# AdaptiveCity/deepdish

Hardware: AMD Instinct MI355X
Metric: end-to-end frames/sec (detect+encode+track) at 640x480 (higher is better)
Workload: dtype i8 (reference: uint8); encoder f16; 1 GPU; SSD-MobileNet-v1 uint8-quantised (300x300) + MARS-64x32x3 + deep_sort on synthetic 640x480 BGR frames, ~20 synthetic detections/frame (BASELINE.json configs[1]); streams_per_gpu=3072, worker_threads_per_gpu=2, parallelism=independent streams, 3072 per GPU in 2 worker groups, weights=seeded synthetic (seed 1234)

## Files before the change

### deepdish_amd/_lib.py

```python
import ctypes
import os
from ctypes import c_int, c_int64, c_double, c_float, c_void_p, c_char_p, POINTER

HERE = os.path.dirname(os.path.abspath(__file__))
LIB_PATH = os.environ.get('DD_LIB') or os.path.join(HERE, 'libdeepdish_hip.so')

P = c_void_p


class DeepDishHipError(RuntimeError):
    pass


SIGNATURES = {
    'dd_last_error': [],
    'dd_version': [],
    'dd_ctx_create': [c_int, POINTER(P)],
    'dd_ctx_destroy': [P],
    'dd_ctx_stream': [P, POINTER(P)],
    'dd_ctx_sync': [P],
    'dd_kf_initiate': [P, P, P, P, P, c_int, P],
    'dd_kf_predict': [P, P, P, P, c_int, P],
    'dd_kf_project': [P, P, P, P, c_int, P, P, P],
    'dd_kf_update': [P, P, P, P, P, c_int, P],
# ... 44 lines not shown
    'dd_ingest_create_jpeg_scaled': [P, c_int, c_int, c_int, c_int, c_int, c_int, c_int, c_int, c_int64, P],
    'dd_ingest_jpeg_put': [P, c_int, c_int, P, c_int64],
    'dd_ingest_create_jpeg_ex': [P, c_int, c_int, c_int, c_int, c_int, c_int, c_int, c_int, c_int, c_int64, P],
    'dd_ingest_status': [P, c_int, P],
    'dd_ingest_destroy': [P],
    'dd_ingest_host_slot': [P, c_int, P, P],
    'dd_ingest_submit': [P, c_int],
    'dd_ingest_wait_uploaded': [P, c_int],
    'dd_ingest_acquire': [P, c_int, P, P],
    'dd_ingest_release': [P, c_int, P],
    'dd_mog2_create': [P, c_int, c_int, c_int, c_int, c_double, c_int, POINTER(P)],
    'dd_mog2_destroy': [P],
    'dd_mog2_state': [P, c_int, P, P, P, P],
    'dd_mog2_apply': [P, P, c_double, P, P, P],
    'dd_mog2_apply_streams': [P, P, P, c_double, P, P, P],
    'dd_mask_box_count': [P, P, c_int, c_int, c_int, P, P, c_int, P, P],
    'dd_net_create': [P, P, c_int, P, c_int64, c_int, POINTER(P)],
    'dd_net_create_shared': [P, P, c_int, P, c_int64, c_int, POINTER(P)],
    'dd_net_activation_bytes': [P, POINTER(c_int64)],
    'dd_net_destroy': [P],
    'dd_net_forward': [P, P, c_int, P],
    'dd_net_output': [P, c_int, POINTER(P), POINTER(c_int), POINTER(c_int), POINTER(c_int), POINTER(c_int),
                      POINTER(c_int)],
    'dd_net_use_graph': [P, c_int],
    'dd_net_input_size': [P, POINTER(c_int), POINTER(c_int)],
    'dd_net_max_batch': [P, POINTER(c_int)],
    'dd_net_last_batch': [P, POINTER(c_int)],
    'dd_net_read': [P, c_int, c_int, P, c_int, P],
    'dd_net_profile': [P, c_int],
    'dd_net_profile_read': [P, P, c_int, POINTER(c_int)],
    'dd_net_op_launches': [P, P, c_int, POINTER(c_int)],
    'dd_net_op_variants': [P, P, c_int, POINTER(c_int)],
    'dd_netq_dwpw_fits': [c_int, c_int, c_int, c_int, c_int, c_int, POINTER(c_int)],
    'dd_ssd_postprocess': [P, P, P, c_int, c_int, c_int, c_float, c_float, P, P, P, P, P],
    'dd_ssd_decode': [P, P, P, c_int, c_int, c_float, P, P, P, P, c_int, P],
    'dd_ssd_postprocess_decoded': [P, P, P, P, P, c_int, c_int, c_float, c_float, P, P, P, P, c_int, P],
    'dd_ssd_regular_nms_decoded': [P, P, P, c_int, c_int, c_int, c_int, c_int, c_int, c_float, c_float, P, P, P, P, c_int, P],
    'dd_ssd_postprocess_regular': [P, P, P, c_int, c_int, c_int, c_int, c_float, c_float, P, P, P, P, c_int, P],
    'dd_ssd_postprocess_regular_u8': [P, P, P, c_int, P, P, P, c_int, c_int, c_int, c_int, c_float, c_float, P, P, P, P, c_int, P],
    'dd_net_ssd_heads_u8': [P, POINTER(P), POINTER(P), POINTER(c_int), POINTER(P), P, POINTER(c_int), POINTER(c_int)],
    'dd_net_ssd_decode': [P, P, c_int, c_float, c_int],
    'dd_net_ssd_decoded': [P, POINTER(P), POINTER(P), POINTER(P), POINTER(P)],
    'dd_net_ssd_decoded_read': [P, c_int, P, P, P, P],
    'dd_net_yolo_decode': [P, c_int],
    'dd_net_yolo_decoded': [P, P, P, P, P],
    'dd_net_yolo_decoded_read': [P, c_int, P, P, P],
    'dd_ssd_detections': [P, P, P, P, c_int, c_int, c_double, c_double, c_double, c_double, P, P, P, P, P],
    'dd_yolov5_decode': [P, P, c_int, c_int, c_float, c_float, c_float, P, P, P, c_int, P, P],
    'dd_yolov5_decode_letterbox': [P, P, c_int, c_int, c_float, c_int, c_int, c_int, c_int, P, P, P, c_int, P, P],
    'dd_pipeline_create': [P, c_int, c_int, c_int, P, P, c_int, c_int, P, c_char_p, c_char_p, c_double, c_double,
                           c_double, c_int, c_int, P, c_int, c_int, POINTER(P)],
    'dd_pipeline_destroy': [P],
    'dd_pipeline_detector_adaptor': [P, c_int],
    'dd_pipeline_ssd_options': [P, c_int, c_float, c_float],
    'dd_pipeline_ssd_regular_nms': [P, c_int],
    'dd_pipeline_detector_skip_frames': [P, c_int],
    'dd_pipeline_detector_letterbox': [P, c_int],
    'dd_pipeline_metric': [P, c_int],
    'dd_pipeline_association': [P, c_int],
    'dd_pipeline_step': [P, P, P, P, P, P],
    'dd_pipeline_step2': [P, P, P, P, P, P, P],
    'dd_pipeline_step3': [P, P, P, P, P, P, P, P, P],
    'dd_pipeline_frames_seen': [P, P],
    'dd_pipeline_present_stats': [P, P],
    'dd_pipeline_detector_skip_streams': [P, P, P],
    'dd_pipeline_skip_stats': [P, P, P],
# ... 97 lines not shown
```

### deepdish_amd/csrc/netsq.hip

```cpp
#include <algorithm>
#include <atomic>
#include <cstdlib>
#include <type_traits>
#include "common.h"
#include "ssd_dev.h"
#include "net_priv.h"
#include "netsq_dev.h"

namespace {


struct QConvP {
    const uint8_t *in; int H, W, c16_in;
    int kh, kw, stride, off_y, off_x;
    int ho, wo, m;
    const i4v *w;
    const int *cbias;
    int kc_per_tap, n_mfrag, mq;
    uint8_t *out; int epi;
    int Ho, Wo, c16_out;
    long long img_bytes_out; int row_bytes, base_off, cout_store;
    int zwc;
    unsigned hw_magic, wo_magic;
    QReq R;
// ... 433 lines not shown
        const u4v v = *reinterpret_cast<const u4v *>(c + sub * 16);
#pragma unroll
        for (int i = 0; i < 16; ++i) {
            const int k = sub * 16 + i;
            const int q = lut[(v[i >> 2] >> (8 * (i & 3))) & 0xffu];
            if (k >= 1 && k < P.n_classes && q > best) { best = q; bi = k - 1; }
        }
    }
#pragma unroll
    for (int o = 4; o > 0; o >>= 1) {
        const int ob = __shfl_xor(best, o, 64), oi = __shfl_xor(bi, o, 64);
        if (ob > best || (ob == best && oi < bi)) { best = ob; bi = oi; }
    }
    if (live && sub == 0) {
#pragma clang fp contract(off)
        const uint8_t *b = P.box + (z * P.n_anchors + a) * 4;
        float r[4], an[4], bx[4];
#pragma unroll
        for (int q = 0; q < 4; ++q) { r[q] = P.box_scale * ((float)b[q] - P.box_zp); an[q] = P.anchors[a * 4 + q]; }
        (void)ssddev::decode_anchor(r, an, 0.f, bx);
        const float sc = P.sc_scale * ((float)best - P.sc_zp);
        const size_t o = z * P.n_anchors + a;
#pragma unroll
        for (int q = 0; q < 4; ++q) P.boxes[o * 4 + q] = bx[q];
        P.score[o] = sc;
        P.cls_out[o] = bi;
        P.keys[o] = sc >= P.thr ? sc : -1.f;
    }
}

struct QDwpwP {
    const uint8_t *in; int H, W;
    int off_y, off_x, ho, wo, hw, tiles_per_frame;
    uint8_t *out; int c16_out;
    const uint2 *dw_a;
    const long long *dw_cq;
    const i4v *w;
    const i4v *w2;
    const int *cbias;
    const long long *cq;
    int zwc, NR;
    int dup;
    unsigned wo_magic, nr_magic, tpf_magic;
    unsigned long long *dbg;
    QReq Rd, Rp;
};

constexpr int QT = 64;

template <int CIN, int COUT, int WP, int STRIDE, int LPT, bool ROWSUM, int MW = 4, int SAT = 0, bool HL = false, int QTT = QT>
__global__ __launch_bounds__((COUT / (16 * MW)) * WP * 64, (COUT / (16 * MW)) * WP <= 2 ? 3 : QTT > 64 ? 4 : 2) void q_dwpw_k(const QDwpwP P, const int n_tiles, const int tiles_per_block) {
    constexpr int WM = COUT / (16 * MW), NW = WM * WP, NT = NW * 64;
    static_assert(MW == 4 || MW == 2, "fragments per wave");
    static_assert(!(HL && ROWSUM), "the split filter needs no row sums");
    constexpr int KC = (CIN + 63) / 64, CINP = KC * 64, C16 = CIN / 16;
    constexpr int FPT = QTT / 16, UNITS = C16 * (FPT / 4);
    static_assert(QTT % 64 == 0 && UNITS % NW == 0, "depthwise units over waves");
    constexpr int CPW = UNITS / NW;
    static_assert(FPT == 4 || CPW == 1, "several units per wave: one fragment quad only");
    constexpr bool KEEP = CPW <= 2, FOLDP = !ROWSUM && KC <= 4 && QTT == 64;
    extern __shared__ __attribute__((aligned(16))) uint8_t smem[];
    const int tid = threadIdx.x, lane = tid & 63, wave = __builtin_amdgcn_readfirstlane(tid >> 6);
    const int fr = lane & 15, fq = lane >> 4;
    const int wm = wave / WP, wp = wave % WP;
    const int RB = (P.W + 2) * CIN, PP = (P.W + 2) * 16;
    uint8_t *opnd = smem;
    int *rowsum = reinterpret_cast<int *>(opnd + QTT * CINP);
    i4v *pinfo = reinterpret_cast<i4v *>(rowsum + 2 * QTT);
    int *cbl = reinterpret_cast<int *>(pinfo + 2 * QTT);
    uint2 *dwa_l = reinterpret_cast<uint2 *>(cbl + COUT);
    long long *dwq_l = reinterpret_cast<long long *>(dwa_l + (KEEP ? 0 : C16 * 64));
    uint8_t *ring = reinterpret_cast<uint8_t *>(dwq_l + (KEEP ? 0 : CIN));

    i4v Wr[MW][KC];
#pragma unroll
    for (int m = 0; m < MW; ++m)
#pragma unroll
        for (int kc = 0; kc < KC; ++kc) Wr[m][kc] = P.w[((size_t)(wm * MW + m) * KC + kc) * 64 + lane];
    const int mg = (wm * MW) / 4, m0 = (wm * MW) % 4;
    unsigned wlm = 0;
    int kcl = -1;
    i4v Wl1[HL ? MW : 1];
    if constexpr (HL) {
// ... 31 lines not shown
    int tap_dx[3];
#pragma unroll
    for (int ks = 0; ks < 3; ++ks) tap_dx[ks] = (min(4 * ks + fq, 8) % 3) * 16;
    const bool row_up0 = fq == 3, row_up1 = fq >= 2;
    auto build_a = [&](int cg, i4v (&Ah)[3], unsigned &lo_w, long long (&Cq)[4], unsigned &lom) {
        const uint2 ab = P.dw_a[cg * 64 + lane];
        lo_w = ab.y;
        lom = (unsigned)__builtin_amdgcn_readfirstlane((int)(ab.y >> 24));
#pragma unroll
        for (int ks = 0; ks < 3; ++ks) {
            const unsigned rh = __builtin_amdgcn_perm(ab.x, ab.x, 0x01010101u * (unsigned)ks);
#pragma unroll
            for (int d = 0; d < 4; ++d) Ah[ks][d] = (int)(rh & dmask[d]);
        }
#pragma unroll
        for (int r = 0; r < 4; ++r) Cq[r] = P.dw_cq[cg * 16 + 4 * fq + r];
    };
    i4v KAh[KEEP ? CPW : 1][3];
    long long KCq[KEEP ? CPW : 1][4];
    unsigned Klom[KEEP ? CPW : 1] = {}, Klow[KEEP ? CPW : 1] = {};
    if constexpr (KEEP) {
#pragma unroll
        for (int ci = 0; ci < CPW; ++ci) build_a((wave * CPW + ci) % C16, KAh[ci], Klow[ci], KCq[ci], Klom[ci]);
    }

    const int t_begin = blockIdx.x * tiles_per_block, t_end = min(n_tiles, t_begin + tiles_per_block);
    if (t_begin >= t_end) return;
    const int Md = P.Rd.M, shd = P.Rd.e - 1, Mp = P.Rp.M, shp = P.Rp.e - 1;
    const long long Cp = P.Rp.C;
    const int lod = P.Rd.lo, hid = P.Rd.hi, lop = P.Rp.lo, hip_ = P.Rp.hi;
    const int out_row = P.c16_out * ((P.wo + 2) * 16);
    const unsigned ring_bytes = (unsigned)P.NR * (unsigned)RB;

    auto tile_rows = [&](int t, int &n, int &q0, int &q1, int &ga, int &gb) {
        n = (int)__umulhi((unsigned)t, P.tpf_magic);
        q0 = (t - n * P.tiles_per_frame) * QTT;
        q1 = min(q0 + QTT, P.hw) - 1;
        const int y0 = (int)__umulhi((unsigned)q0, P.wo_magic), y1 = (int)__umulhi((unsigned)q1, P.wo_magic);
        ga = n * (P.H + 2) + y0 * STRIDE + P.off_y;
        gb = n * (P.H + 2) + y1 * STRIDE + P.off_y + 2;
    };
    auto geometry = [&](int n, int q0, int q1, int ga, int buf) {
        const int q = q0 + tid;
        const int qc = min(q, q1);
        const int y = (int)__umulhi((unsigned)qc, P.wo_magic), x = qc - __mul24(y, P.wo);
        const int y0 = (int)__umulhi((unsigned)q0, P.wo_magic);
        const int sa = ga - (int)__umulhi((unsigned)ga, P.nr_magic) * P.NR;
        int s0 = sa + (y - y0) * STRIDE;
        s0 = s0 >= P.NR ? s0 - P.NR : s0;
        const int s1 = s0 + 1 == P.NR ? 0 : s0 + 1, s2 = s1 + 1 == P.NR ? 0 : s1 + 1;
        const int col = (x * STRIDE + P.off_x) * 16;
        const unsigned po = q <= q1 ? (unsigned)__mul24(n * (P.ho + 2) + y + 1, out_row) + (unsigned)(x + 1) * 16u : 0xffffffffu;
        pinfo[buf * QTT + tid] = i4v{__mul24(s0, RB) + col, __mul24(s1, RB) + col, __mul24(s2, RB) + col, (int)po};
    };
    auto load_rows_sync = [&](int lo, int hi) {
        if (hi < lo) return;
        const unsigned nb = (unsigned)(hi - lo + 1) * RB;
        const uint8_t *src = P.in + (size_t)lo * RB;
        for (unsigned idx = tid * 16u; idx < nb; idx += NT * 16u) {
            const unsigned row = idx / (unsigned)RB, off = idx - row * RB;
            *reinterpret_cast<u4v *>(ring + (size_t)((lo + row) % P.NR) * RB + off) = *reinterpret_cast<const u4v *>(src + idx);
        }
    };
    auto dw_planes = [&](int gbuf, int rsb) __attribute__((always_inline)) {
        int rs[4] = {0, 0, 0, 0};
        constexpr int FB = QTT > 64 ? 2 : 4;
        constexpr bool TAP_ONCE = FB == 4;
        int tapoff[3][4];
        const int fb = 4 * ((wave * CPW) / C16);
        auto taps = [&](int f0, int nfr) __attribute__((always_inline)) {
#pragma unroll
            for (int f = 0; f < 4; ++f) {
                if (f < f0 || f >= f0 + nfr) continue;
                const i4v pi = pinfo[gbuf * QTT + 16 * (fb + f) + fr];
                tapoff[0][f] = (row_up0 ? pi[1] : pi[0]) + tap_dx[0];
                tapoff[1][f] = (row_up1 ? pi[2] : pi[1]) + tap_dx[1];
                tapoff[2][f] = pi[2] + tap_dx[2];
            }
        };
        if constexpr (TAP_ONCE) taps(0, 4);
        auto plane = [&](int unit, int ci) __attribute__((always_inline)) {
            const int cg = unit % C16;
            const int pofs = cg * PP;
            uint2 ab = make_uint2(0u, 0u);
            if constexpr (!KEEP) ab = dwa_l[cg * 64 + lane];
// ... 133 lines not shown
                if (fq == 0) atomicAdd(&rowsum[rsb * QTT + 16 * (fb + f) + fr], v);
            }
        }
    };
    auto glds16 = [&](const uint8_t *g, const uint8_t *l) {
        unsigned keep;
        const unsigned dst = (unsigned)(uintptr_t)(const __attribute__((address_space(3))) uint8_t *)l;
        asm volatile("s_mov_b32 %0, m0\n\ts_mov_b32 m0, %2\n\ts_nop 0\n\tglobal_load_lds_dwordx4 %1, off\n\ts_mov_b32 m0, %0"
                     : "=&s"(keep) : "v"(g), "s"(dst) : "memory");
    };
    auto pf_issue = [&](int lo, int hi) {
        if (hi < lo) return;
        const unsigned nb = (unsigned)(hi - lo + 1) * (unsigned)RB;
        const uint8_t *src = P.in + (size_t)lo * RB;
        const unsigned base = (unsigned)(lo - (int)__umulhi((unsigned)lo, P.nr_magic) * P.NR) * (unsigned)RB;
#pragma unroll
        for (int i = 0; i < LPT; ++i) {
            const unsigned cb = (unsigned)(i * NW + wave) * 1024u;
            if (cb < nb) {
                unsigned a = base + cb;
                a = a >= ring_bytes ? a - ring_bytes : a;
                const unsigned idx = cb + (unsigned)lane * 16u;
                const uint8_t *g = src + idx;
                if (a + 1024u <= ring_bytes) {
                    if (idx < nb) glds16(g, ring + a);
                } else {
                    const bool first = a + (unsigned)lane * 16u < ring_bytes;
                    if (idx < nb && first) glds16(g, ring + a);
                    if (idx < nb && !first) glds16(g, ring + (int)(a - ring_bytes));
                }
            }
        }
    };
    auto matrix = [&](int q0, int q1, int gbuf, int rsb) __attribute__((always_inline)) {
        const int nf = (q1 - q0) / 16 + 1;
        constexpr int KB = KC < 4 ? KC : 4;
        i4v b[KB];
        if (wp < nf) {
            const uint8_t *bp = opnd + ((size_t)fq * QTT + 16 * wp + fr) * 16;
#pragma unroll
            for (int kc = 0; kc < KB; ++kc) b[kc] = *reinterpret_cast<const i4v *>(bp + (size_t)kc * 4 * QTT * 16);
        }
        for (int f = wp; f < nf; f += WP) {
            i4v acc[MW];
#pragma unroll
            for (int m = 0; m < MW; ++m) {
                if constexpr (FOLDP) acc[m] = i4v{0, 0, 0, 0};
                else acc[m] = *reinterpret_cast<const i4v *>(cbl + 64 * mg + 16 * fq + 4 * (m0 + m));
            }
            const uint8_t *bp = opnd + ((size_t)fq * QTT + 16 * f + fr) * 16;
#pragma unroll
            for (int k0 = 0; k0 < KC; k0 += KB) {
#pragma unroll
                for (int kc = 0; kc < KB; ++kc) {
#pragma unroll
                    for (int m = 0; m < MW; ++m) acc[m] = __builtin_amdgcn_mfma_i32_16x16x64_i8(Wr[m][k0 + kc], b[kc], acc[m], 0, 0, 0);
                    if (HL && ((wlm >> (k0 + kc)) & 1u)) {
                        if (k0 + kc == kcl) {
#pragma unroll
                            for (int m = 0; m < MW; ++m) acc[m] = __builtin_amdgcn_mfma_i32_16x16x64_i8(Wl1[m], b[kc], acc[m], 0, 0, 0);
                        } else {
#pragma unroll
                            for (int m = 0; m < MW; ++m) acc[m] = __builtin_amdgcn_mfma_i32_16x16x64_i8(P.w2[((size_t)(wm * MW + m) * KC + (k0 + kc)) * 64 + lane], b[kc], acc[m], 0, 0, 0);
                        }
                    }
                }
                if (k0 + KB < KC) {
#pragma unroll
                    for (int kc = 0; kc < KB; ++kc) b[kc] = *reinterpret_cast<const i4v *>(bp + (size_t)(k0 + KB + kc) * 4 * QTT * 16);
                }
            }
            if (f + WP < nf) {
                const uint8_t *bn = opnd + ((size_t)fq * QTT + 16 * (f + WP) + fr) * 16;
#pragma unroll
                for (int kc = 0; kc < KB; ++kc) b[kc] = *reinterpret_cast<const i4v *>(bn + (size_t)kc * 4 * QTT * 16);
            }
            const int rsv = ROWSUM ? rowsum[rsb * QTT + 16 * f + fr] * P.zwc : 0;
            const unsigned po = (unsigned)pinfo[gbuf * QTT + 16 * f + fr][3];
            unsigned o[MW];
#pragma unroll
            for (int m = 0; m < MW; ++m) {
                if constexpr (FOLDP)
                    o[m] = 0x80808080u ^ q_requant_pack4<SAT>(acc[m][0], acc[m][1], acc[m][2], acc[m][3], Mp, CP[m][0], CP[m][1], CP[m][2], CP[m][3], shp, lop, hip_);
                else
                    o[m] = 0x80808080u ^ q_requant_pack4<SAT>(acc[m][0] + rsv, acc[m][1] + rsv, acc[m][2] + rsv, acc[m][3] + rsv, Mp, Cp, Cp, Cp, Cp, shp, lop, hip_);
            }
            if (po != 0xffffffffu) {
                uint8_t *dst = P.out + po + (size_t)(4 * mg + fq) * ((P.wo + 2) * 16) + 4 * m0;
                if constexpr (MW == 4) *reinterpret_cast<u4v *>(dst) = u4v{o[0], o[1], o[2], o[3]};
                else *reinterpret_cast<uint2 *>(dst) = make_uint2(o[0], o[1]);
            }
        }
    };
    int n, q0, q1, ga, gb;
    tile_rows(t_begin, n, q0, q1, ga, gb);
    load_rows_sync(ga, gb);
    if (tid < QTT) geometry(n, q0, q1, ga, t_begin & 1);
    int loaded_hi = gb;
    __syncthreads();
    unsigned long long st[6] = {0, 0, 0, 0, 0, 0}, tprev = P.dbg ? __builtin_amdgcn_s_memtime() : 0ull;
#define Q_STAMP(k) do { if (P.dbg) { const unsigned long long now_ = __builtin_amdgcn_s_memtime(); st[k] += now_ - tprev; tprev = now_; } } while (0)

    for (int t = t_begin; t < t_end; ++t) {
        int lo = 0, hi = -1, e_hi = -1;
        int n2 = 0, q02 = 0, q12 = 0, ga2 = 0, gb2 = 0;
        if (t + 1 < t_end) {
            tile_rows(t + 1, n2, q02, q12, ga2, gb2);
            lo = max(loaded_hi + 1, ga2);
            hi = gb2;
            e_hi = min(hi, ga + P.NR - 1);
            loaded_hi = max(loaded_hi, gb2);
        }
        pf_issue(lo, e_hi);
        const int cur = t & 1;
        dw_planes(cur, cur);
        Q_STAMP(0);
        __builtin_amdgcn_s_waitcnt(0xc07f);
        __builtin_amdgcn_s_barrier();
        Q_STAMP(1);
        pf_issue(max(lo, e_hi + 1), hi);
        if (tid < QTT) {
            if (ROWSUM) rowsum[(cur ^ 1) * QTT + tid] = 0;
            if (t + 1 < t_end) geometry(n2, q02, q12, ga2, cur ^ 1);
        }
        matrix(q0, q1, cur, cur);
        Q_STAMP(2);
        {
            const int nf_t = (q1 - q0) / 16 + 1, ns = nf_t > wp ? (nf_t - wp + WP - 1) / WP : 0;
            if (ns >= 4) __builtin_amdgcn_s_waitcnt(0x0f74);
            else if (ns == 3) __builtin_amdgcn_s_waitcnt(0x0f73);
            else if (ns == 2) __builtin_amdgcn_s_waitcnt(0x0f72);
            else if (ns == 1) __builtin_amdgcn_s_waitcnt(0x0f71);
            else __builtin_amdgcn_s_waitcnt(0x0f70);
        }
        Q_STAMP(3);
        __builtin_amdgcn_s_waitcnt(0xc07f);
        __builtin_amdgcn_s_barrier();
        Q_STAMP(4);
        n = n2; q0 = q02; q1 = q12; ga = ga2;
    }
#undef Q_STAMP
    if (P.dbg && lane == 0) for (int k = 0; k < 5; ++k) P.dbg[((size_t)blockIdx.x * NW + wave) * 8 + k] = st[k];
}



enum { QV_CONV = 1, QV_PWS = 2, QV_DW = 3, QV_DWM = 4, QV_DWPW = 5, QV_CONV0 = 6, QV_ADD = 7, QV_DECODE = 8 };

void dwpw_plan(int H, int W, int ho, int wo, int stride, int off_y, int cin, int nt, int qt, int *NR, int *lpt) {
    const int hw = ho * wo, tpf = dd_ceil_div(hw, qt), RB = (W + 2) * cin;
    int span = 0, hi = 0, mx = 0;
    for (int n = 0; n < 2; ++n)
        for (int k = 0; k < tpf; ++k) {
            const int q0 = k * qt, q1 = std::min(q0 + qt, hw) - 1;
            const int ga = n * (H + 2) + (q0 / wo) * stride + off_y, gb = n * (H + 2) + (q1 / wo) * stride + off_y + 2;
            span = std::max(span, gb - ga + 1);
            if (n || k) { const int lo = std::max(hi + 1, ga); mx = std::max(mx, gb - lo + 1); }
            hi = std::max(hi, gb);
        }
    *NR = span;
    *lpt = (int)(((long long)mx * RB + (long long)nt * 16 - 1) / ((long long)nt * 16));
}

template <int CIN, int COUT, int WP, int STRIDE, int LPT, int EXTRA = 0, int MW = 4, int QTT = QT>
int launch_q_dwpw(hipStream_t s, QDwpwP &P, int nimg, int device, bool *ok, bool dry = false, int *variant = nullptr, bool dry_split = false) {
    constexpr int NW = (COUT / (16 * MW)) * WP, NT = NW * 64, CINP = (CIN + 63) / 64 * 64;
    int lpt = 0;
    P.tiles_per_frame = dd_ceil_div(P.hw, QTT);
    dwpw_plan(P.H, P.W, P.ho, P.wo, STRIDE, P.off_y, CIN, NT, QTT, &P.NR, &lpt);
    P.NR += EXTRA;
    const int RB = (P.W + 2) * CIN;
    constexpr bool KEEP = ((CIN / 16) * (QTT / 64)) / NW <= 2;
    const size_t lds = (size_t)P.NR * RB + (size_t)QTT * CINP + (size_t)2 * QTT * sizeof(int) + 2 * QTT * 16 + COUT * sizeof(int) + (KEEP ? 0 : (CIN / 16) * 64 * 8 + CIN * 8);
    P.wo_magic = (unsigned)((1ull << 32) / (unsigned)P.wo) + 1u;
    P.nr_magic = (unsigned)((1ull << 32) / (unsigned)P.NR) + 1u;
    P.tpf_magic = (unsigned)((1ull << 32) / (unsigned)P.tiles_per_frame) + 1u;
    const long long lim24 = 1ll << 23;
    *ok = (long long)nimg * P.tiles_per_frame * P.tiles_per_frame < (1ll << 32) && (long long)P.hw * P.wo < (1ll << 32) &&
          (long long)(nimg + 1) * (P.H + 2) * P.NR < (1ll << 32) && lpt <= LPT && lds <= 160 * 1024 && (long long)LPT * NT * 16 + (long long)P.NR * RB < (1ll << 32) &&
          RB < lim24 && (long long)P.c16_out * (P.wo + 2) * 16 < lim24 && (long long)(nimg + 1) * (P.ho + 2) < lim24 && P.hw < lim24;
    if (!*ok) return DD_OK;
    constexpr bool CAN_HL = CIN <= 128;
    const bool hl = dry ? dry_split : P.w2 != nullptr;
    if (hl && !CAN_HL) { *ok = false; return DD_OK; }
    if (dry) return DD_OK;
    const bool rsum = P.zwc != 0 && !hl;
    const int sat = P.Rd.lo == 0 && P.Rd.hi == 255 && P.Rp.lo == 0 && P.Rp.hi == 255 ? (P.Rd.e <= 8 && P.Rp.e <= 8 ? 2 : 1) : 0;
#define DD_QK(R_, S_, H_) q_dwpw_k<CIN, COUT, WP, STRIDE, LPT, R_, MW, S_, (H_) && CAN_HL, QTT>
#define DD_QS(R_, H_) (sat == 2 ? &DD_QK(R_, 2, H_) : sat == 1 ? &DD_QK(R_, 1, H_) : &DD_QK(R_, 0, H_))
    void (*kern)(const QDwpwP, const int, const int) = hl ? DD_QS(false, true) : rsum ? DD_QS(true, false) : DD_QS(false, false);
    if (variant) *variant = QV_DWPW | (CIN / 32) << 4 | (COUT / 64) << 9 | STRIDE << 13 | (QTT / 64) << 15 | (hl ? 2 : rsum ? 1 : P.dup ? 3 : 0) << 17 | sat << 19;
    static DevOnce once;
    const int rc = once.run(device, [&]() -> int {
        for (const void *f : {reinterpret_cast<const void *>(&DD_QK(false, 0, true)), reinterpret_cast<const void *>(&DD_QK(false, 1, true)), reinterpret_cast<const void *>(&DD_QK(false, 2, true)),
                              reinterpret_cast<const void *>(&DD_QK(true, 0, false)), reinterpret_cast<const void *>(&DD_QK(true, 1, false)), reinterpret_cast<const void *>(&DD_QK(true, 2, false)),
                              reinterpret_cast<const void *>(&DD_QK(false, 0, false)), reinterpret_cast<const void *>(&DD_QK(false, 1, false)), reinterpret_cast<const void *>(&DD_QK(false, 2, false))})
            DD_HIP(hipFuncSetAttribute(f, hipFuncAttributeMaxDynamicSharedMemorySize, 160 * 1024));
        return DD_OK;
    });
#undef DD_QS
#undef DD_QK
    if (rc != DD_OK) return rc;
    static std::atomic<int> per_cu_cache[64];
    int per_cu = per_cu_cache[device & 63].load(std::memory_order_relaxed);
    if (per_cu == 0) {
        int nb = 0;
        DD_HIP(hipOccupancyMaxActiveBlocksPerMultiprocessor(&nb, reinterpret_cast<const void *>(kern), NT, lds));
        per_cu = std::max(1, std::min(8, nb));
        per_cu_cache[device & 63].store(per_cu, std::memory_order_relaxed);
    }
    const int n_tiles = nimg * P.tiles_per_frame;
    const int blocks = std::min(n_tiles, per_cu * 256);
    const int tpb = dd_ceil_div(n_tiles, blocks);
    const dim3 grid((unsigned)dd_ceil_div(n_tiles, tpb));
    static const bool stamps = dd_env_int("DD_Q_STAMPS", 0) != 0;
    const size_t n_st = (size_t)grid.x * NW * 8;
    if (stamps) { DD_HIP(hipMalloc(&P.dbg, n_st * 8)); DD_HIP(hipMemsetAsync(P.dbg, 0, n_st * 8, s)); }
    hipLaunchKernelGGL(kern, grid, dim3(NT), lds, s, P, n_tiles, tpb);
    DD_LAUNCH_CHECK();
    if (stamps) {
        std::vector<unsigned long long> h(n_st);
        DD_HIP(hipStreamSynchronize(s));
        DD_HIP(hipMemcpy(h.data(), P.dbg, n_st * 8, hipMemcpyDeviceToHost));
        DD_HIP(hipFree(P.dbg));
        double sum[5] = {0, 0, 0, 0, 0};
        for (size_t w = 0; w < n_st / 8; ++w) for (int k = 0; k < 5; ++k) sum[k] += (double)h[w * 8 + k];
        const double nw = (double)(n_st / 8) * tpb;
        fprintf(stderr, "q_dwpw_k<%d,%d,%d> %d blocks/CU %d tiles/block: cycles per wave and tile: depthwise %.0f  barrier A %.0f  matrix stage %.0f  ring write %.0f  barrier B %.0f\n",
                CIN, COUT, STRIDE, per_cu, tpb, sum[0] / nw, sum[1] / nw, sum[2] / nw, sum[3] / nw, sum[4] / nw);
    }
    return DD_OK;
}

int dwpw_dispatch(hipStream_t s, QDwpwP &Q, int nc, int dev, int cin, int cout, int stride, bool *ok, bool dry, int *variant, bool dry_split = false) {
    static const int qt128 = dd_env_int("DD_Q_QT128", 1);
    *ok = false;
#define DD_QB(CIN_, COUT_, WP_, S_, LPT_) launch_q_dwpw<CIN_, COUT_, WP_, S_, LPT_>(s, Q, nc, dev, ok, dry, variant, dry_split)
    if (cin == 32 && cout == 64 && stride == 1) return qt128 ? launch_q_dwpw<32, 64, 4, 1, 6, 0, 4, 128>(s, Q, nc, dev, ok, dry, variant, dry_split) : DD_QB(32, 64, 2, 1, 8);
    if (cin == 64 && cout == 128 && stride == 2) return DD_QB(64, 128, 2, 2, 8);
    if (cin == 128 && cout == 128 && stride == 1) return DD_QB(128, 128, 2, 1, 8);
    if (cin == 128 && cout == 256 && stride == 2) return DD_QB(128, 256, 2, 2, 8);
    if (cin == 256 && cout == 256 && stride == 1) return DD_QB(256, 256, 2, 1, 6);
    if (cin == 256 && cout == 512 && stride == 2) return DD_QB(256, 512, 1, 2, 12);
    if (cin == 512 && cout == 512 && stride == 1) return DD_QB(512, 512, 1, 1, 8);
// ... 252 lines not shown
    const unsigned u = (unsigned)it, w = (unsigned)P.W, c = (unsigned)P.c16, h = (unsigned)P.H;
    const unsigned x = u % w, q1 = u / w, p = q1 % c, q2 = q1 / c, y = q2 % h, n = q2 / h;
    const size_t off = (((size_t)n * (P.H + 2) + y + 1) * P.c16 + p) * (size_t)(P.W + 2) * 16 + (size_t)(x + 1) * 16;
    const u4v a = *reinterpret_cast<const u4v *>(P.a + off), b = *reinterpret_cast<const u4v *>(P.b + off);
    u4v o;
#pragma unroll
    for (int d = 0; d < 4; ++d) {
        const unsigned av = a[d] ^ 0x80808080u, bv = b[d] ^ 0x80808080u;
        unsigned wv = 0;
#pragma unroll
        for (int r = 0; r < 4; ++r) wv |= (unsigned)q_add_u8((int)((av >> (8 * r)) & 0xffu), (int)((bv >> (8 * r)) & 0xffu), P.A) << (8 * r);
        o[d] = wv ^ 0x80808080u;
    }
    *reinterpret_cast<u4v *>(P.out + off) = o;
}

}

int netq_prepare(dd_net *) { return DD_OK; }

int dd_netq_dwpw_fits(int cin, int cout, int stride, int h, int w, int split_filter, int *fits_host) {
    DD_REQUIRE(fits_host && cin > 0 && cout > 0 && (stride == 1 || stride == 2) && h > 0 && w > 0 && h < (1 << 20) && w < (1 << 20), DD_E_ARG,
               "dd_netq_dwpw_fits: %d -> %d channels, stride %d, %d x %d", cin, cout, stride, h, w);
    if ((long long)((h + stride - 1) / stride) * ((w + stride - 1) / stride) >= (1ll << 23)) { *fits_host = 0; return DD_OK; }
    QDwpwP Q;
    memset(&Q, 0, sizeof(Q));
    Q.H = h; Q.W = w; Q.ho = (h + stride - 1) / stride; Q.wo = (w + stride - 1) / stride; Q.hw = Q.ho * Q.wo;
    Q.off_y = 1 - std::max((Q.ho - 1) * stride + 3 - h, 0) / 2; Q.off_x = 1 - std::max((Q.wo - 1) * stride + 3 - w, 0) / 2;
    Q.c16_out = cout / 16;
    bool ok = false;
    const int rc = dwpw_dispatch(nullptr, Q, 1, 0, cin, cout, stride, &ok, true, nullptr, split_filter != 0);
    if (rc != DD_OK) return rc;
    *fits_host = ok ? 1 : 0;
    return DD_OK;
}

int netq_run_op(dd_net *net, int i, const int32_t *o, const uint8_t *input, int nimg, hipStream_t s, int *handled) {
    const int kind = o[W_KIND], src = o[W_SRC], dst = o[W_DST];
    *handled = kind >= OP_QCONV0 && kind <= OP_QADD;
    if (!*handled) return DD_OK;
    auto base = [&](int t) -> uint8_t * { return static_cast<uint8_t *>(net->bufs[net->tensors[t].buf]); };
    const TensorDesc *ts = src >= 0 ? &net->tensors[src] : nullptr;
    const TensorDesc *td = dst >= 0 ? &net->tensors[dst] : nullptr;
    char *W = net->d_weights;
    int variant_none = 0;
    int *const variant = i < (int)net->op_variant.size() ? &net->op_variant[i] : &variant_none;
    switch (kind) {
        case OP_QCONV0: {
            QConv0P P;
            P.src = input; P.H = net->in_h; P.W = net->in_w; P.total_bytes = (long long)nimg * P.H * P.W * 3;
            P.stride = o[W_STRIDE]; P.pad_t = o[W_PAD_T]; P.pad_l = o[W_PAD_L]; P.ho = td->h; P.wo = td->w; P.m = nimg * P.ho * P.wo;
            P.w = reinterpret_cast<const i4v *>(W + (size_t)(uint32_t)o[W_W_OFF]);
            P.w2 = o[W_AFF_OFF] ? reinterpret_cast<const i4v *>(W + (size_t)(uint32_t)o[W_AFF_OFF]) : nullptr;
            P.cq = reinterpret_cast<const long long *>(W + (size_t)(uint32_t)o[W_Q_CQ_OFF]);
            P.out = base(dst); P.in_zp = o[W_Q_IN_ZP]; P.zwc = o[W_Q_ZWC]; P.R = make_req(o);
            P.out_bytes = (long long)nimg * (P.ho + 2) * 2 * (P.wo + 2) * 16;
            DD_REQUIRE(td->w >= 16, DD_E_ARG, "dd_net_forward: uint8 first layer: output narrower than a fragment");
            DD_REQUIRE(td->pad == 1 && td->cs == 32 && o[W_COUT] == 32 && (reinterpret_cast<uintptr_t>(input) & 3) == 0 && (P.total_bytes & 3) == 0 && !P.R.linear && P.R.e >= 1,
                       DD_E_ARG, "dd_net_forward: uint8 first layer: 32 channels into a bordered tensor from a 4-byte aligned batch");
            DD_REQUIRE(o[W_Q_CQ_OFF] != 0, DD_E_ARG, "dd_net_forward: uint8 first layer: no folded requantisation constants in the program");
            const long long in_img = (long long)P.H * P.W * 3, out_img = (long long)(P.ho + 2) * 2 * (P.wo + 2) * 16, lim31 = (1ll << 31) - 17;
            long long lim = std::min(lim31 / in_img, lim31 / out_img);
            if (in_img % 4) lim &= ~3ll;
            DD_REQUIRE(lim >= 1, DD_E_CAPACITY, "dd_net_forward: uint8 first layer: one frame beyond 31-bit offsets");
            const long long n_chunks = (nimg + lim - 1) / lim;
            long long chunk = (nimg + n_chunks - 1) / n_chunks;
// ... 260 lines not shown
```

### include/deepdish_hip.h

```cpp
#ifndef DEEPDISH_HIP_H
#define DEEPDISH_HIP_H

#include <stdint.h>

#ifdef __cplusplus
extern "C" {
#endif

#define DD_OK            0
#define DD_E_ARG        -1
#define DD_E_HIP        -2
#define DD_E_STATE      -3
#define DD_E_CAPACITY   -4

#define DD_FEATURE_DIM 128

typedef struct dd_ctx dd_ctx;
typedef struct dd_tracker dd_tracker;
typedef struct dd_net dd_net;
typedef struct dd_pipeline dd_pipeline;

const char *dd_last_error(void);
int dd_version(void);

// ... 136 lines not shown
int dd_mog2_state(dd_mog2 *m, int stream_index, float *weight_host, float *variance_host, float *mean_host, uint8_t *nmodes_host);
int dd_mog2_reset_streams(dd_mog2 *m, const int *streams_host, int n, void *stream);
int dd_mask_box_count(dd_ctx *ctx, const uint8_t *mask, int n_streams, int height, int width, const int *boxes_xywh_host,
                      const int *box_stream_host, int n_boxes, int *counts_host, void *stream);

int dd_gather_frames(dd_ctx *ctx, const uint8_t *src_dev, int n_src, int64_t frame_bytes, const int *idx_host, int n, uint8_t *dst_dev,
                     void *stream);

int dd_feature_rows_carry(dd_ctx *ctx, const float *fresh_dev, int64_t fresh_rows, const float *store_dev, int64_t store_rows,
                          float *rows_out_dev, int64_t out_rows, float *store_out_dev, int64_t store_out_rows, const int *table_host,
                          int n_streams, void *stream);

int dd_net_create(dd_ctx *ctx, const int32_t *program_host, int n_words, const void *weights_host,
                  int64_t n_weight_bytes, int max_batch, dd_net **out);
int dd_net_create_shared(dd_ctx *ctx, const int32_t *program_host, int n_words, const void *weights_host,
                         int64_t n_weight_bytes, int max_batch, dd_net **out);
int dd_net_activation_bytes(dd_net *net, int64_t *out_host);
int dd_net_destroy(dd_net *net);
int dd_net_forward(dd_net *net, const uint8_t *input, int n, void *stream);
int dd_net_output(dd_net *net, int tensor, void **dev_ptr_host, int *h_host, int *w_host, int *c_host,
                  int *cs_host, int *dtype_host);

int dd_net_use_graph(dd_net *net, int enable);
int dd_net_input_size(dd_net *net, int *h_host, int *w_host);
int dd_net_max_batch(dd_net *net, int *out_host);
int dd_net_last_batch(dd_net *net, int *out_host);
int dd_net_read(dd_net *net, int tensor, int n, void *dst, int dst_on_device, void *stream);

int dd_net_profile(dd_net *net, int enable);
int dd_net_profile_read(dd_net *net, float *ms_host, int cap, int *n_ops_host);
int dd_net_op_launches(dd_net *net, int32_t *codes_host, int cap, int *n_ops_host);
int dd_net_op_variants(dd_net *net, int32_t *codes_host, int cap, int *n_ops_host);
int dd_netq_dwpw_fits(int cin, int cout, int stride, int h, int w, int split_filter, int *fits_host);

int dd_ssd_postprocess(dd_ctx *ctx, const float *raw, const float *anchors, int n_anchors,
                       int n_classes, int max_det, float score_thr, float iou_thr,
                       float *boxes, float *classes, float *scores, int *count, void *stream);

int dd_ssd_decode(dd_ctx *ctx, const float *raw, const float *anchors, int n_anchors, int n_classes, float score_thr,
                  float *boxes, float *scores, int *classes, float *keys, int batch, void *stream);
int dd_ssd_postprocess_decoded(dd_ctx *ctx, const float *dec_boxes, const float *dec_scores, const int *dec_classes,
                               const float *dec_keys, int n_anchors, int max_det, float score_thr, float iou_thr,
                               float *boxes, float *classes, float *scores, int *count, int batch, void *stream);
int dd_net_ssd_decode(dd_net *net, const float *anchors_host, int n_anchors, float score_thr, int enable);
int dd_net_ssd_decoded(dd_net *net, float **boxes_dev, float **scores_dev, int **classes_dev, float **keys_dev);
int dd_net_ssd_decoded_read(dd_net *net, int n, float *boxes_host, float *scores_host, int *classes_host, float *keys_host);

int dd_ssd_regular_nms_decoded(dd_ctx *ctx, const float *dec_boxes, const float *scores_in, int score_ld, int first_class_col,
                               int n_anchors, int n_classes, int max_det, int detections_per_class, float score_thr, float iou_thr,
                               float *boxes, float *classes, float *scores, int *count, int batch, void *stream);
int dd_ssd_postprocess_regular(dd_ctx *ctx, const float *raw, const float *anchors, int n_anchors, int n_classes, int max_det,
                               int detections_per_class, float score_thr, float iou_thr, float *boxes, float *classes, float *scores,
                               int *count, int batch, void *stream);
int dd_ssd_postprocess_regular_u8(dd_ctx *ctx, const uint8_t *box_q, const uint8_t *cls_q, int cls_stride, const uint8_t *logistic_table,
                                  const float *quant4_host, const float *anchors, int n_anchors, int n_classes, int max_det,
                                  int detections_per_class, float score_thr, float iou_thr, float *boxes, float *classes, float *scores,
                                  int *count, int batch, void *stream);
int dd_net_ssd_heads_u8(dd_net *net, const uint8_t **box_q_dev, const uint8_t **cls_q_dev, int *cls_stride_host,
                        const uint8_t **logistic_table_dev, float *quant4_host, int *n_anchors_host, int *n_classes_host);

int dd_net_yolo_decode(dd_net *net, int enable);
int dd_net_yolo_decoded(dd_net *net, float **boxes, float **conf, int **classes, int *rows);
int dd_net_yolo_decoded_read(dd_net *net, int n, float *boxes_host, float *conf_host, int *classes_host);

int dd_ssd_detections(dd_ctx *ctx, const float *boxes, const float *classes, const float *scores, int batch,
                      int max_det, double confidence, double iou_thr, double img_w, double img_h, double *out_boxes,
// ... 194 lines not shown
```

Baseline: 118,500 frames/s.

## Let fused depthwise-pointwise tiles span frame boundaries to remove partial tiles

Adds a SPAN variant of the quantised depthwise+pointwise kernel. Pixel tiles of fixed size run over the flattened batch of frames instead of restarting at each frame, so small feature maps (e.g. 19x19, 10x10) no longer leave a partially filled tile per frame. A host planner computes the row-ring size and prefetch depth needed when a tile crosses a frame. The variant is used only if LDS occupancy stays the same. The cost is extra per-pixel geometry logic and more template instantiations. A tile-count query API is also added.

```diff
diff --git a/deepdish_amd/_lib.py b/deepdish_amd/_lib.py
--- a/deepdish_amd/_lib.py
+++ b/deepdish_amd/_lib.py
@@ -100,6 +100,7 @@
     'dd_net_op_launches': [P, P, c_int, POINTER(c_int)],
     'dd_net_op_variants': [P, P, c_int, POINTER(c_int)],
     'dd_netq_dwpw_fits': [c_int, c_int, c_int, c_int, c_int, c_int, POINTER(c_int)],
+    'dd_netq_dwpw_tiles': [c_int, c_int, c_int, c_int, c_int, c_int, POINTER(c_int), POINTER(c_int)],
     'dd_ssd_postprocess': [P, P, P, c_int, c_int, c_int, c_float, c_float, P, P, P, P, P],
     'dd_ssd_decode': [P, P, P, c_int, c_int, c_float, P, P, P, P, c_int, P],
     'dd_ssd_postprocess_decoded': [P, P, P, P, P, c_int, c_int, c_float, c_float, P, P, P, P, c_int, P],
diff --git a/deepdish_amd/csrc/netsq.hip b/deepdish_amd/csrc/netsq.hip
--- a/deepdish_amd/csrc/netsq.hip
+++ b/deepdish_amd/csrc/netsq.hip
@@ -489,6 +489,8 @@
 struct QDwpwP {
     const uint8_t *in; int H, W;
     int off_y, off_x, ho, wo, hw, tiles_per_frame;
+    int span, total;
+    int n_tiles;
     uint8_t *out; int c16_out;
     const uint2 *dw_a;
     const long long *dw_cq;
@@ -505,7 +507,7 @@
 
 constexpr int QT = 64;
 
-template <int CIN, int COUT, int WP, int STRIDE, int LPT, bool ROWSUM, int MW = 4, int SAT = 0, bool HL = false, int QTT = QT>
+template <int CIN, int COUT, int WP, int STRIDE, int LPT, bool ROWSUM, int MW = 4, int SAT = 0, bool HL = false, int QTT = QT, bool SPAN = false>
 __global__ __launch_bounds__((COUT / (16 * MW)) * WP * 64, (COUT / (16 * MW)) * WP <= 2 ? 3 : QTT > 64 ? 4 : 2) void q_dwpw_k(const QDwpwP P, const int n_tiles, const int tiles_per_block) {
     constexpr int WM = COUT / (16 * MW), NW = WM * WP, NT = NW * 64;
     static_assert(MW == 4 || MW == 2, "fragments per wave");
@@ -603,25 +605,50 @@
     const int out_row = P.c16_out * ((P.wo + 2) * 16);
     const unsigned ring_bytes = (unsigned)P.NR * (unsigned)RB;
 
-    auto tile_rows = [&](int t, int &n, int &q0, int &q1, int &ga, int &gb) {
-        n = (int)__umulhi((unsigned)t, P.tpf_magic);
-        q0 = (t - n * P.tiles_per_frame) * QTT;
-        q1 = min(q0 + QTT, P.hw) - 1;
-        const int y0 = (int)__umulhi((unsigned)q0, P.wo_magic), y1 = (int)__umulhi((unsigned)q1, P.wo_magic);
+    auto tile_at = [&](int t, int &n, int &q0) {
+        if constexpr (SPAN) {
+            const unsigned g0 = (unsigned)t * (unsigned)QTT;
+            n = (int)(g0 / (unsigned)P.hw);
+            q0 = (int)(g0 - (unsigned)n * (unsigned)P.hw);
+        } else {
+            n = (int)__umulhi((unsigned)t, P.tpf_magic);
+            q0 = (t - n * P.tiles_per_frame) * QTT;
+        }
+    };
+    auto tile_next = [&](int t1, int &n, int &q0) {
+        if constexpr (SPAN) {
+            q0 += QTT;
+            if (q0 >= P.hw) { q0 -= P.hw; ++n; }
+        } else {
+            tile_at(t1, n, q0);
+        }
+    };
+    auto tile_rows = [&](int n, int q0, int &cnt, int &nl, int &ga, int &gb) {
+        cnt = SPAN ? min(QTT, P.total - (n * P.hw + q0)) : min(QTT, P.hw - q0);
+        int ql = q0 + cnt - 1;
+        nl = n;
+        if constexpr (SPAN) {
+            if (ql >= P.hw) { ql -= P.hw; ++nl; }
+        }
+        const int y0 = (int)__umulhi((unsigned)q0, P.wo_magic), y1 = (int)__umulhi((unsigned)ql, P.wo_magic);
         ga = n * (P.H + 2) + y0 * STRIDE + P.off_y;
-        gb = n * (P.H + 2) + y1 * STRIDE + P.off_y + 2;
+        gb = nl * (P.H + 2) + y1 * STRIDE + P.off_y + 2;
     };
-    auto geometry = [&](int n, int q0, int q1, int ga, int buf) {
-        const int q = q0 + tid;
-        const int qc = min(q, q1);
-        const int y = (int)__umulhi((unsigned)qc, P.wo_magic), x = qc - __mul24(y, P.wo);
+    auto geometry = [&](int n, int q0, int cnt, int nl, int ga, int buf) {
+        int q = q0 + min(tid, cnt - 1), dn = 0, on = 0;
+        if constexpr (SPAN) {
+            if (nl != n) {
+                if (q >= P.hw) { q -= P.hw; dn = P.H + 2; on = P.ho + 2; }
+            }
+        }
+        const int y = (int)__umulhi((unsigned)q, P.wo_magic), x = q - __mul24(y, P.wo);
         const int y0 = (int)__umulhi((unsigned)q0, P.wo_magic);
         const int sa = ga - (int)__umulhi((unsigned)ga, P.nr_magic) * P.NR;
-        int s0 = sa + (y - y0) * STRIDE;
+        int s0 = sa + dn + (y - y0) * STRIDE;
         s0 = s0 >= P.NR ? s0 - P.NR : s0;
         const int s1 = s0 + 1 == P.NR ? 0 : s0 + 1, s2 = s1 + 1 == P.NR ? 0 : s1 + 1;
         const int col = (x * STRIDE + P.off_x) * 16;
-        const unsigned po = q <= q1 ? (unsigned)__mul24(n * (P.ho + 2) + y + 1, out_row) + (unsigned)(x + 1) * 16u : 0xffffffffu;
+        const unsigned po = tid < cnt ? (unsigned)__mul24(n * (P.ho + 2) + on + y + 1, out_row) + (unsigned)(x + 1) * 16u : 0xffffffffu;
         pinfo[buf * QTT + tid] = i4v{__mul24(s0, RB) + col, __mul24(s1, RB) + col, __mul24(s2, RB) + col, (int)po};
     };
     auto load_rows_sync = [&](int lo, int hi) {
@@ -821,8 +848,8 @@
             }
         }
     };
-    auto matrix = [&](int q0, int q1, int gbuf, int rsb) __attribute__((always_inline)) {
-        const int nf = (q1 - q0) / 16 + 1;
+    auto matrix = [&](int cnt, int gbuf, int rsb) __attribute__((always_inline)) {
+        const int nf = (cnt - 1) / 16 + 1;
         constexpr int KB = KC < 4 ? KC : 4;
         i4v b[KB];
         if (wp < nf) {
@@ -881,10 +908,11 @@
             }
         }
     };
-    int n, q0, q1, ga, gb;
-    tile_rows(t_begin, n, q0, q1, ga, gb);
+    int n, q0, cnt, nl, ga, gb;
+    tile_at(t_begin, n, q0);
+    tile_rows(n, q0, cnt, nl, ga, gb);
     load_rows_sync(ga, gb);
-    if (tid < QTT) geometry(n, q0, q1, ga, t_begin & 1);
+    if (tid < QTT) geometry(n, q0, cnt, nl, ga, t_begin & 1);
     int loaded_hi = gb;
     __syncthreads();
     unsigned long long st[6] = {0, 0, 0, 0, 0, 0}, tprev = P.dbg ? __builtin_amdgcn_s_memtime() : 0ull;
@@ -892,9 +920,10 @@
 
     for (int t = t_begin; t < t_end; ++t) {
         int lo = 0, hi = -1, e_hi = -1;
-        int n2 = 0, q02 = 0, q12 = 0, ga2 = 0, gb2 = 0;
+        int n2 = n, q02 = q0, cnt2 = 0, nl2 = 0, ga2 = 0, gb2 = 0;
         if (t + 1 < t_end) {
-            tile_rows(t + 1, n2, q02, q12, ga2, gb2);
+            tile_next(t + 1, n2, q02);
+            tile_rows(n2, q02, cnt2, nl2, ga2, gb2);
             lo = max(loaded_hi + 1, ga2);
             hi = gb2;
             e_hi = min(hi, ga + P.NR - 1);
@@ -910,12 +939,12 @@
         pf_issue(max(lo, e_hi + 1), hi);
         if (tid < QTT) {
             if (ROWSUM) rowsum[(cur ^ 1) * QTT + tid] = 0;
-            if (t + 1 < t_end) geometry(n2, q02, q12, ga2, cur ^ 1);
-        }
-        matrix(q0, q1, cur, cur);
+            if (t + 1 < t_end) geometry(n2, q02, cnt2, nl2, ga2, cur ^ 1);
+        }
+        matrix(cnt, cur, cur);
         Q_STAMP(2);
         {
-            const int nf_t = (q1 - q0) / 16 + 1, ns = nf_t > wp ? (nf_t - wp + WP - 1) / WP : 0;
+            const int nf_t = (cnt - 1) / 16 + 1, ns = nf_t > wp ? (nf_t - wp + WP - 1) / WP : 0;
             if (ns >= 4) __builtin_amdgcn_s_waitcnt(0x0f74);
             else if (ns == 3) __builtin_amdgcn_s_waitcnt(0x0f73);
             else if (ns == 2) __builtin_amdgcn_s_waitcnt(0x0f72);
@@ -926,7 +955,7 @@
         __builtin_amdgcn_s_waitcnt(0xc07f);
         __builtin_amdgcn_s_barrier();
         Q_STAMP(4);
-        n = n2; q0 = q02; q1 = q12; ga = ga2;
+        n = n2; q0 = q02; cnt = cnt2; ga = ga2;
     }
 #undef Q_STAMP
     if (P.dbg && lane == 0) for (int k = 0; k < 5; ++k) P.dbg[((size_t)blockIdx.x * NW + wave) * 8 + k] = st[k];
@@ -951,6 +980,34 @@
     *lpt = (int)(((long long)mx * RB + (long long)nt * 16 - 1) / ((long long)nt * 16));
 }
 
+void dwpw_plan_span(int H, int W, int ho, int wo, int stride, int off_y, int cin, int nt, int qt, int nimg, int *NR, int *lpt) {
+    const int hw = ho * wo, RB = (W + 2) * cin;
+    int g = hw, r = qt;
+    while (r) { const int x = g % r; g = r; r = x; }
+    const int frames = std::min(nimg, qt / g + 1);
+    struct Key { int H, W, ho, wo, stride, off_y, qt, frames, NR, mx; };
+    thread_local std::vector<Key> memo;
+    int span = 0, mx = 0;
+    bool hit = false;
+    for (const Key &k : memo)
+        if (k.H == H && k.W == W && k.ho == ho && k.wo == wo && k.stride == stride && k.off_y == off_y && k.qt == qt && k.frames == frames) { span = k.NR; mx = k.mx; hit = true; break; }
+    if (!hit) {
+        const long long total = (long long)frames * hw;
+        int hi = 0;
+        for (long long g0 = 0; g0 < total; g0 += qt) {
+            const long long g1 = std::min(g0 + qt, total) - 1;
+            const int n0 = (int)(g0 / hw), q0 = (int)(g0 - (long long)n0 * hw), n1 = (int)(g1 / hw), q1 = (int)(g1 - (long long)n1 * hw);
+            const int ga = n0 * (H + 2) + (q0 / wo) * stride + off_y, gb = n1 * (H + 2) + (q1 / wo) * stride + off_y + 2;
+            span = std::max(span, gb - ga + 1);
+            if (g0) { const int lo = std::max(hi + 1, ga); mx = std::max(mx, gb - lo + 1); }
+            hi = std::max(hi, gb);
+        }
+        if (memo.size() < 64) memo.push_back(Key{H, W, ho, wo, stride, off_y, qt, frames, span, mx});
+    }
+    *NR = span;
+    *lpt = (int)(((long long)mx * RB + (long long)nt * 16 - 1) / ((long long)nt * 16));
+}
+
 template <int CIN, int COUT, int WP, int STRIDE, int LPT, int EXTRA = 0, int MW = 4, int QTT = QT>
 int launch_q_dwpw(hipStream_t s, QDwpwP &P, int nimg, int device, bool *ok, bool dry = false, int *variant = nullptr, bool dry_split = false) {
     constexpr int NW = (COUT / (16 * MW)) * WP, NT = NW * 64, CINP = (CIN + 63) / 64 * 64;
@@ -960,33 +1017,50 @@
     P.NR += EXTRA;
     const int RB = (P.W + 2) * CIN;
     constexpr bool KEEP = ((CIN / 16) * (QTT / 64)) / NW <= 2;
-    const size_t lds = (size_t)P.NR * RB + (size_t)QTT * CINP + (size_t)2 * QTT * sizeof(int) + 2 * QTT * 16 + COUT * sizeof(int) + (KEEP ? 0 : (CIN / 16) * 64 * 8 + CIN * 8);
+    constexpr size_t lds_rest = (size_t)QTT * CINP + (size_t)2 * QTT * sizeof(int) + 2 * QTT * 16 + COUT * sizeof(int) + (KEEP ? 0 : (CIN / 16) * 64 * 8 + CIN * 8);
+    size_t lds = (size_t)P.NR * RB + lds_rest;
     P.wo_magic = (unsigned)((1ull << 32) / (unsigned)P.wo) + 1u;
-    P.nr_magic = (unsigned)((1ull << 32) / (unsigned)P.NR) + 1u;
     P.tpf_magic = (unsigned)((1ull << 32) / (unsigned)P.tiles_per_frame) + 1u;
     const long long lim24 = 1ll << 23;
-    *ok = (long long)nimg * P.tiles_per_frame * P.tiles_per_frame < (1ll << 32) && (long long)P.hw * P.wo < (1ll << 32) &&
-          (long long)(nimg + 1) * (P.H + 2) * P.NR < (1ll << 32) && lpt <= LPT && lds <= 160 * 1024 && (long long)LPT * NT * 16 + (long long)P.NR * RB < (1ll << 32) &&
-          RB < lim24 && (long long)P.c16_out * (P.wo + 2) * 16 < lim24 && (long long)(nimg + 1) * (P.ho + 2) < lim24 && P.hw < lim24;
+    auto fits = [&](int NR_, int lpt_, size_t lds_) {
+        return (long long)nimg * P.tiles_per_frame * QTT < (1ll << 31) && (long long)nimg * P.tiles_per_frame * P.tiles_per_frame < (1ll << 32) && (long long)P.hw * P.wo < (1ll << 32) &&
+               (long long)(nimg + 1) * (P.H + 2) * NR_ < (1ll << 32) && lpt_ <= LPT && lds_ <= 160 * 1024 && (long long)LPT * NT * 16 + (long long)NR_ * RB < (1ll << 32) &&
+               RB < lim24 && (long long)P.c16_out * (P.wo + 2) * 16 < lim24 && (long long)(nimg + 1) * (P.ho + 2) < lim24 && P.hw < lim24;
+    };
+    *ok = fits(P.NR, lpt, lds);
     if (!*ok) return DD_OK;
+    static const bool span_env = dd_env_int("DD_Q_TILE_SPAN", 1) != 0;
+    P.span = 0;
+    P.total = nimg * P.hw;
+    if (span_env && P.hw >= QTT && nimg > 1) {
+        int nr_s = 0, lpt_s = 0;
+        dwpw_plan_span(P.H, P.W, P.ho, P.wo, STRIDE, P.off_y, CIN, NT, QTT, nimg, &nr_s, &lpt_s);
+        nr_s += EXTRA;
+        const size_t lds_s = (size_t)nr_s * RB + lds_rest;
+        if (fits(nr_s, lpt_s, lds_s) && (160 * 1024) / lds_s == (160 * 1024) / lds) { P.span = 1; P.NR = nr_s; lds = lds_s; }
+    }
+    P.nr_magic = (unsigned)((1ull << 32) / (unsigned)P.NR) + 1u;
+    P.n_tiles = P.span ? dd_ceil_div(P.total, QTT) : nimg * P.tiles_per_frame;
     constexpr bool CAN_HL = CIN <= 128;
     const bool hl = dry ? dry_split : P.w2 != nullptr;
     if (hl && !CAN_HL) { *ok = false; return DD_OK; }
     if (dry) return DD_OK;
     const bool rsum = P.zwc != 0 && !hl;
     const int sat = P.Rd.lo == 0 && P.Rd.hi == 255 && P.Rp.lo == 0 && P.Rp.hi == 255 ? (P.Rd.e <= 8 && P.Rp.e <= 8 ? 2 : 1) : 0;
-#define DD_QK(R_, S_, H_) q_dwpw_k<CIN, COUT, WP, STRIDE, LPT, R_, MW, S_, (H_) && CAN_HL, QTT>
-#define DD_QS(R_, H_) (sat == 2 ? &DD_QK(R_, 2, H_) : sat == 1 ? &DD_QK(R_, 1, H_) : &DD_QK(R_, 0, H_))
-    void (*kern)(const QDwpwP, const int, const int) = hl ? DD_QS(false, true) : rsum ? DD_QS(true, false) : DD_QS(false, false);
+#define DD_QK(R_, S_, H_, T_) q_dwpw_k<CIN, COUT, WP, STRIDE, LPT, R_, MW, S_, (H_) && CAN_HL, QTT, T_>
+#define DD_QS(R_, H_, T_) (sat == 2 ? &DD_QK(R_, 2, H_, T_) : sat == 1 ? &DD_QK(R_, 1, H_, T_) : &DD_QK(R_, 0, H_, T_))
+    void (*kern)(const QDwpwP, const int, const int) = P.span ? (hl ? DD_QS(false, true, true) : rsum ? DD_QS(true, false, true) : DD_QS(false, false, true))
+                                                              : (hl ? DD_QS(false, true, false) : rsum ? DD_QS(true, false, false) : DD_QS(false, false, false));
     if (variant) *variant = QV_DWPW | (CIN / 32) << 4 | (COUT / 64) << 9 | STRIDE << 13 | (QTT / 64) << 15 | (hl ? 2 : rsum ? 1 : P.dup ? 3 : 0) << 17 | sat << 19;
     static DevOnce once;
     const int rc = once.run(device, [&]() -> int {
-        for (const void *f : {reinterpret_cast<const void *>(&DD_QK(false, 0, true)), reinterpret_cast<const void *>(&DD_QK(false, 1, true)), reinterpret_cast<const void *>(&DD_QK(false, 2, true)),
-                              reinterpret_cast<const void *>(&DD_QK(true, 0, false)), reinterpret_cast<const void *>(&DD_QK(true, 1, false)), reinterpret_cast<const void *>(&DD_QK(true, 2, false)),
-                              reinterpret_cast<const void *>(&DD_QK(false, 0, false)), reinterpret_cast<const void *>(&DD_QK(false, 1, false)), reinterpret_cast<const void *>(&DD_QK(false, 2, false))})
+#define DD_QF(R_, S_, H_) reinterpret_cast<const void *>(&DD_QK(R_, S_, H_, false)), reinterpret_cast<const void *>(&DD_QK(R_, S_, H_, true))
+        for (const void *f : {DD_QF(false, 0, true), DD_QF(false, 1, true), DD_QF(false, 2, true), DD_QF(true, 0, false), DD_QF(true, 1, false), DD_QF(true, 2, false),
+                              DD_QF(false, 0, false), DD_QF(false, 1, false), DD_QF(false, 2, false)})
             DD_HIP(hipFuncSetAttribute(f, hipFuncAttributeMaxDynamicSharedMemorySize, 160 * 1024));
         return DD_OK;
     });
+#undef DD_QF
 #undef DD_QS
 #undef DD_QK
     if (rc != DD_OK) return rc;
@@ -998,7 +1072,7 @@
         per_cu = std::max(1, std::min(8, nb));
         per_cu_cache[device & 63].store(per_cu, std::memory_order_relaxed);
     }
-    const int n_tiles = nimg * P.tiles_per_frame;
+    const int n_tiles = P.n_tiles;
     const int blocks = std::min(n_tiles, per_cu * 256);
     const int tpb = dd_ceil_div(n_tiles, blocks);
     const dim3 grid((unsigned)dd_ceil_div(n_tiles, tpb));
@@ -1317,6 +1391,23 @@
     const int rc = dwpw_dispatch(nullptr, Q, 1, 0, cin, cout, stride, &ok, true, nullptr, split_filter != 0);
     if (rc != DD_OK) return rc;
     *fits_host = ok ? 1 : 0;
+    return DD_OK;
+}
+
+int dd_netq_dwpw_tiles(int cin, int cout, int stride, int h, int w, int frames, int *tiles_host, int *span_host) {
+    DD_REQUIRE(tiles_host && span_host && cin > 0 && cout > 0 && (stride == 1 || stride == 2) && h > 0 && w > 0 && h < (1 << 20) && w < (1 << 20) && frames > 0, DD_E_ARG,
+               "dd_netq_dwpw_tiles: %d -> %d channels, stride %d, %d x %d, %d frames", cin, cout, stride, h, w, frames);
+    *tiles_host = 0; *span_host = 0;
+    if ((long long)((h + stride - 1) / stride) * ((w + stride - 1) / stride) >= (1ll << 23)) return DD_OK;
+    QDwpwP Q;
+    memset(&Q, 0, sizeof(Q));
+    Q.H = h; Q.W = w; Q.ho = (h + stride - 1) / stride; Q.wo = (w + stride - 1) / stride; Q.hw = Q.ho * Q.wo;
+    Q.off_y = 1 - std::max((Q.ho - 1) * stride + 3 - h, 0) / 2; Q.off_x = 1 - std::max((Q.wo - 1) * stride + 3 - w, 0) / 2;
+    Q.c16_out = cout / 16;
+    bool ok = false;
+    const int rc = dwpw_dispatch(nullptr, Q, frames, 0, cin, cout, stride, &ok, true, nullptr, false);
+    if (rc != DD_OK) return rc;
+    if (ok) { *tiles_host = Q.n_tiles; *span_host = Q.span; }
     return DD_OK;
 }
 
diff --git a/include/deepdish_hip.h b/include/deepdish_hip.h
--- a/include/deepdish_hip.h
+++ b/include/deepdish_hip.h
@@ -192,6 +192,7 @@
 int dd_net_op_launches(dd_net *net, int32_t *codes_host, int cap, int *n_ops_host);
 int dd_net_op_variants(dd_net *net, int32_t *codes_host, int cap, int *n_ops_host);
 int dd_netq_dwpw_fits(int cin, int cout, int stride, int h, int w, int split_filter, int *fits_host);
+int dd_netq_dwpw_tiles(int cin, int cout, int stride, int h, int w, int frames, int *tiles_host, int *span_host);
 
 int dd_ssd_postprocess(dd_ctx *ctx, const float *raw, const float *anchors, int n_anchors,
                        int n_classes, int max_det, float score_thr, float iou_thr,
```

Result: slower. 111,500 frames/s (-5.9%).
